# Ghostish/Open3DSOT

Measured on AMD Instinct MI355X. Metric: template/search pairs/sec (fwd+bwd), BAT KITTI-Car 512/1024 pts, higher is better.
Workload: dtype f32; 1 GPU; BAT_Car.yaml KITTI-Car, template 512 / search 1024 pts, batch 48 per GPU, fwd+bwd+Adam, fp32; global_batch=48, parallelism=dp1, fused_kernels=True, hip_graph=True, rccl_world_size=1

## Files before the change

### open3dsot_amd/csrc/mlp.hip

```cpp
#include "mlp_common.hpp"

#include <mutex>
#include <unordered_set>

bool o3d_direct_ok(int M, int K, int P);
int o3d_direct_fwd(const float* X, const float* W, const float* in_scale, const float* in_shift, int B, int Cin,
                   int Cout, int P, float* Y, float* part, const float* stat_c, const float* w, const int32_t* meta,
                   long start1, int tile, hipStream_t st);
int o3d_direct_dgrad(const float* dN, const float* pk, int ns,
                     const float* Y, const float* A1, const float* A2, const float* A3, const float* Wt, int B,
                     int Cin, int Cout, int P, const float* Yprev, const float* scale_p, const float* shift_p,
                     const float* mean_p, float* dNprev, float* part, const float* w, const int32_t* meta,
                     long start1, int tile, hipStream_t st);

namespace {


constexpr int BN_POS = 128;
constexpr int BK = 16;
constexpr int LDMK = BK + 4;
constexpr int WBK = 32;
constexpr int WLD = WBK + 4;

template <int CH, bool A_MK, bool B_MK>
// ... 623 lines not shown
        const int p = (ch - (int)b * chunks_per_b) * WBK + 4 * c4;
#pragma unroll
        for (int i = 0; i < 4; ++i) {
            const int co = co0 + r0 + 32 * i;
            if (co < a.Cout) ra[i] = load_dy_raw<POOLED>(a.dy, b, co, a.Cout, a.P, p);
            const int ci = ci0 + r0 + 32 * i;
            float4 v = make_float4(0.f, 0.f, 0.f, 0.f);
            float c0 = 0.f, c1 = 0.f;
            if (ci < a.Cin) {
                v = *reinterpret_cast<const float4*>(&a.X[(b * a.Cin + ci) * a.P + p]);
                if (XFORM) { c0 = a.in_scale[ci]; c1 = a.in_shift[ci]; }
            }
            rb[i] = v; rc0[i] = c0; rc1[i] = c1;
        }
    };
    auto store_chunk = [&](int buf) {
#pragma unroll
        for (int i = 0; i < 4; ++i) {
            const int co = co0 + r0 + 32 * i;
            *reinterpret_cast<float4*>(&As(buf)[(r0 + 32 * i) * WLD + 4 * c4]) =
                co < a.Cout ? finish_dy<POOLED>(ra[i]) : make_float4(0.f, 0.f, 0.f, 0.f);
            const int ci = ci0 + r0 + 32 * i;
            float4 v = rb[i];
            if (XFORM) {
                if (ci < a.Cin) {
                    const float sc = rc0[i], sh = rc1[i];
                    v.x = fmaxf(fmaf(v.x, sc, sh), 0.f); v.y = fmaxf(fmaf(v.y, sc, sh), 0.f);
                    v.z = fmaxf(fmaf(v.z, sc, sh), 0.f); v.w = fmaxf(fmaf(v.w, sc, sh), 0.f);
                }
            }
            *reinterpret_cast<float4*>(&Bs(buf)[(r0 + 32 * i) * WLD + 4 * c4]) = v;
        }
    };

    f32x16 acc[2][2];
#pragma unroll
    for (int i = 0; i < 2; ++i)
#pragma unroll
        for (int j = 0; j < 2; ++j)
#pragma unroll
            for (int r = 0; r < 16; ++r) acc[i][j][r] = 0.f;

    if (c_begin < c_end) {
        load_chunk(c_begin);
        store_chunk(0);
        __syncthreads();
        for (int ch = c_begin; ch < c_end; ++ch) {
            const int t = ch - c_begin;
            if (ch + 1 < c_end) load_chunk(ch + 1);
            mma_chunk<WBK, true, true>(As(t & 1), WLD, Bs(t & 1), WLD, wm0, wn0, l31, h, acc);
            if (ch + 1 < c_end) store_chunk((t + 1) & 1);
            __syncthreads();
        }
    }
    float* dst = a.part + (long)slice * a.Cout * a.Cin;
#pragma unroll
    for (int tm = 0; tm < 2; ++tm)
#pragma unroll
        for (int r = 0; r < 16; ++r) {
            const int co = co0 + wm0 + 32 * tm + acc_row(r, h);
            if (co >= a.Cout) continue;
#pragma unroll
            for (int tn = 0; tn < 2; ++tn) {
                const int ci = ci0 + wn0 + 32 * tn + l31;
                if (ci < a.Cin) dst[(long)co * a.Cin + ci] = acc[tm][tn][r];
            }
        }
}

__global__ __launch_bounds__(256) void wgrad_reduce_kernel(const float* __restrict__ part, int nslices,
                                                           int per, long n, float* __restrict__ out) {
    const long i = (long)blockIdx.x * 256 + threadIdx.x;
    if (i >= n) return;
    const int z0 = blockIdx.y * per;
    int z1 = z0 + per;
    if (z1 > nslices) z1 = nslices;
    float s = 0.f;
#pragma unroll 8
    for (int z = z0; z < z1; ++z) s += part[(long)z * n + i];
    out[(long)blockIdx.y * n + i] = s;
}

__global__ __launch_bounds__(256) void wgrad_reduce1_kernel(const float* __restrict__ part, int nslices, long n,
                                                            float* __restrict__ out) {
    __shared__ float sh[8][32];
    const int col = threadIdx.x & 31, grp = threadIdx.x >> 5;
    const long i = (long)blockIdx.x * 32 + col;
    const int per = (nslices + 7) / 8, z0 = grp * per;
    int z1 = z0 + per;
    if (z1 > nslices) z1 = nslices;
    float s0 = 0.f, s1 = 0.f, s2 = 0.f, s3 = 0.f;
    if (i < n) {
        int z = z0;
        for (; z + 3 < z1; z += 4) {
            s0 += part[(long)z * n + i]; s1 += part[(long)(z + 1) * n + i];
            s2 += part[(long)(z + 2) * n + i]; s3 += part[(long)(z + 3) * n + i];
        }
        for (; z < z1; ++z) s0 += part[(long)z * n + i];
    }
    sh[grp][col] = (s0 + s1) + (s2 + s3);
    __syncthreads();
    if (grp == 0 && i < n) {
        float t = 0.f;
#pragma unroll
        for (int g = 0; g < 8; ++g) t += sh[g][col];
        out[i] = t;
    }
}

template <typename K, typename... A>
int launch(K kernel, dim3 grid, dim3 block, size_t lds, hipStream_t s, A... args) {
    if (lds > 48 * 1024) {
        static std::mutex mu;
        static std::unordered_set<const void*> done;
        std::lock_guard<std::mutex> lock(mu);
        const void* key = reinterpret_cast<const void*>(kernel);
        if (!done.count(key)) {
            if (hipFuncSetAttribute(key, hipFuncAttributeMaxDynamicSharedMemorySize, (int)lds) != hipSuccess)
                return O3D_ELAUNCH;
            done.insert(key);
        }
    }
    hipLaunchKernelGGL(kernel, grid, block, lds, s, args...);
    return o3d_launch_status();
}

inline size_t fwd_lds(int BM) { return sizeof(float) * (2 * BM * LDMK + 2 * BK * BN_POS); }
inline size_t dgrad_lds(int BM) {
    size_t stage = sizeof(float) * (2 * BK * BM + 2 * BK * BN_POS), red = sizeof(float) * 4 * BM;
    return stage > red ? stage : red;
}

template <bool XFORM>
int launch_fwd(const FwdArgs& a, hipStream_t s) {
    const int tiles = a.B * (a.P / BN_POS);
    if (a.Cout > 128) {
        return launch(conv_fwd_kernel<256, XFORM>, dim3(tiles, o3d_cdiv(a.Cout, 256)), dim3(512),
                      fwd_lds(256), s, a);
    } else if (a.Cout > 64) {
        return launch(conv_fwd_kernel<128, XFORM>, dim3(tiles, 1), dim3(256), fwd_lds(128), s, a);
    }
    return launch(conv_fwd_kernel<64, XFORM>, dim3(tiles, 1), dim3(128), fwd_lds(64), s, a);
}

template <bool POOLED, int EPI>
int launch_dgrad(const DgradArgs& a, hipStream_t s) {
    const int tiles = a.B * (a.P / BN_POS);
    if (a.M > 128) {
        return launch(conv_dgrad_kernel<256, POOLED, EPI>, dim3(tiles, o3d_cdiv(a.M, 256)), dim3(512),
                      dgrad_lds(256), s, a);
    } else if (a.M > 64) {
        return launch(conv_dgrad_kernel<128, POOLED, EPI>, dim3(tiles, 1), dim3(256), dgrad_lds(128), s, a);
    }
    return launch(conv_dgrad_kernel<64, POOLED, EPI>, dim3(tiles, 1), dim3(128), dgrad_lds(64), s, a);
}

}

extern "C" int o3d_mlp_conv_fwd(const float* X, const float* W, const float* in_scale,
                                const float* in_shift, int B, int Cin, int Cout, int P, float* Y,
                                float* part, const float* stat_c, void* stream) {
    if (B <= 0 || Cin <= 0 || Cout <= 0 || P <= 0 || P % BN_POS != 0 || !X || !W || !Y) return O3D_EINVAL;
    if (o3d_direct_ok(Cout, Cin, P) && (in_scale == nullptr) == (in_shift == nullptr))
        return o3d_direct_fwd(X, W, in_scale, in_shift, B, Cin, Cout, P, Y, part, stat_c, nullptr, nullptr, 0,
                              part ? 128 : o3d_direct_tile((long)B * P, Cout, 0), o3d_stream(stream));
    FwdArgs a = {};
    a.X = X; a.W = W; a.Y = Y; a.in_scale = in_scale; a.in_shift = in_shift; a.part = part; a.stat_c = stat_c;
    a.B = B; a.Cin = Cin; a.Cout = Cout; a.P = P;
// ... 60 lines not shown
}

extern "C" int o3d_pool_bwd_partials_split(const float* dOut, const float* out, const float* yarg, const float* mean,
                                           int C, int npoint, int nsplit, float* part, const int32_t* arg, float* pk,
                                           void* stream) {
    if (C <= 0 || npoint <= 0 || nsplit <= 0 || nsplit > 64 || !dOut || !out || !yarg || !mean || !part || (pk && !arg))
        return O3D_EINVAL;
    hipLaunchKernelGGL(pool_bwd_partials_split_kernel, dim3(C, nsplit), dim3(256), 0, o3d_stream(stream), dOut, out, yarg,
                       mean, C, npoint, part, arg, reinterpret_cast<float2*>(pk));
    return o3d_launch_status();
}

static int fill_dy(DyArgs& d, const float* dN, const float* dOut, const float* out, const int32_t* arg,
                   const float* Y, const float* A1, const float* A2, const float* A3, int ns) {
    if (!Y || !A1 || !A2 || !A3) return O3D_EINVAL;
    if (!dN && (!dOut || !out || !arg || ns <= 0 || ns % 4 != 0)) return O3D_EINVAL;
    d.dN = dN; d.dOut = dOut; d.out = out; d.arg = arg; d.Y = Y; d.A1 = A1; d.A2 = A2; d.A3 = A3;
    d.ns = ns > 0 ? ns : 4;
    return O3D_OK;
}

extern "C" int o3d_mlp_conv_dgrad(const float* dN, const float* dOut, const float* out, const int32_t* arg,
                                  int ns, const float* Y, const float* A1, const float* A2, const float* A3,
                                  const float* W, int B, int Cin, int Cout, int P,
                                  const float* Yprev, const float* scale_p, const float* shift_p,
                                  const float* mean_p, float* dNprev, float* part, void* stream) {
    if (B <= 0 || Cin <= 0 || Cout <= 0 || P <= 0 || P % BN_POS != 0 || !W || !Yprev || !scale_p ||
        !shift_p || !mean_p || !dNprev || !part)
        return O3D_EINVAL;
    DgradArgs a = {};
    if (fill_dy(a.dy, dN, dOut, out, arg, Y, A1, A2, A3, ns) != O3D_OK) return O3D_EINVAL;
    a.W = W; a.B = B; a.Cin = Cin; a.Cout = Cout; a.P = P; a.c_lo = 0; a.M = Cin;
    a.Yprev = Yprev; a.scale_p = scale_p; a.shift_p = shift_p; a.mean_p = mean_p; a.dNprev = dNprev; a.part = part;
    return dN ? launch_dgrad<false, 0>(a, o3d_stream(stream)) : launch_dgrad<true, 0>(a, o3d_stream(stream));
}

extern "C" int o3d_mlp_conv_dgrad_wt(const float* dN, const float* dOut, const float* out, const int32_t* arg,
                                     int ns, const float* Y, const float* A1, const float* A2, const float* A3,
                                     const float* W, const float* Wt, const float* pk, int B, int Cin, int Cout,
                                     int P, const float* Yprev, const float* scale_p, const float* shift_p,
                                     const float* mean_p, float* dNprev, float* part, void* stream) {
    if (Wt && o3d_direct_ok(Cin, Cout, P) && B > 0 && Yprev && scale_p && shift_p && mean_p && dNprev && part &&
        Y && A1 && A2 && A3 && (dN || (pk && ns > 0 && ns % 4 == 0)))
        return o3d_direct_dgrad(dN, pk, ns, Y, A1, A2, A3, Wt, B, Cin, Cout, P, Yprev, scale_p, shift_p,
                                mean_p, dNprev, part, nullptr, nullptr, 0, 128, o3d_stream(stream));
    return o3d_mlp_conv_dgrad(dN, dOut, out, arg, ns, Y, A1, A2, A3, W, B, Cin, Cout, P, Yprev, scale_p, shift_p,
                              mean_p, dNprev, part, stream);
}

extern "C" int o3d_mlp_conv_fwd_c(const float* X, const float* W, const float* in_scale, const float* in_shift,
                                  int Cin, int Cout, long ldp, const float* w, const int32_t* meta, long start1,
                                  int tile, float* Y, float* part, const float* stat_c, void* stream) {
    if (!X || !W || !Y || !w || !meta || !in_scale || !in_shift || ldp <= 0 || ldp > 0x7fffffff ||
        !o3d_direct_ok(Cout, Cin, (int)ldp) || (tile != 64 && tile != 128))
        return O3D_EINVAL;
    return o3d_direct_fwd(X, W, in_scale, in_shift, 1, Cin, Cout, (int)ldp, Y, part, stat_c, w, meta, start1, tile,
                          o3d_stream(stream));
}

extern "C" int o3d_mlp_conv_dgrad_c(const float* dN, const float* Y, const float* A1, const float* A2,
                                    const float* A3, const float* Wt, int Cin, int Cout, long ldp, const float* w,
                                    const int32_t* meta, long start1, int tile, const float* Yprev,
                                    const float* scale_p,
                                    const float* shift_p, const float* mean_p, float* dNprev, float* part,
                                    void* stream) {
    if (!dN || !Y || !A1 || !A2 || !A3 || !Wt || !w || !meta || !Yprev || !scale_p || !shift_p || !mean_p ||
        !dNprev || !part || ldp <= 0 || ldp > 0x7fffffff || !o3d_direct_ok(Cin, Cout, (int)ldp) ||
        (tile != 64 && tile != 128))
        return O3D_EINVAL;
    return o3d_direct_dgrad(dN, nullptr, 4, Y, A1, A2, A3, Wt, 1, Cin, Cout, (int)ldp, Yprev, scale_p, shift_p,
                            mean_p, dNprev, part, w, meta, start1, tile, o3d_stream(stream));
}

extern "C" int o3d_mlp_conv_dgrad_plain(const float* dN, const float* Y, const float* A1, const float* A2,
                                        const float* A3, const float* W, int B, int Cin, int Cout, int P,
                                        float* dX, void* stream) {
    if (B <= 0 || Cin <= 0 || Cout <= 0 || P <= 0 || P % BN_POS != 0 || !W || !dN || !dX) return O3D_EINVAL;
    DgradArgs a = {};
    if (fill_dy(a.dy, dN, nullptr, nullptr, nullptr, Y, A1, A2, A3, 4) != O3D_OK) return O3D_EINVAL;
    a.W = W; a.B = B; a.Cin = Cin; a.Cout = Cout; a.P = P; a.c_lo = 0; a.M = Cin; a.dNprev = dX;
    return launch_dgrad<false, 2>(a, o3d_stream(stream));
}

void o3d_wgrad_reduce(const float* part, int nslices, long n, float* dW, hipStream_t s) {
    hipLaunchKernelGGL(wgrad_reduce1_kernel, dim3(o3d_cdiv(n, 32)), dim3(256), 0, s, part, nslices, n, dW);
}

extern "C" int o3d_mlp_conv_wgrad(const float* dN, const float* dOut, const float* out, const int32_t* arg,
                                  int ns, const float* Y, const float* A1, const float* A2, const float* A3,
                                  const float* X, const float* in_scale, const float* in_shift,
                                  int B, int Cin, int Cout, int P, int nslices, float* part, float* dW,
                                  void* stream) {
    if (B <= 0 || Cin <= 0 || Cout <= 0 || P <= 0 || P % WBK != 0 || nslices <= 0 || !X || !part || !dW)
        return O3D_EINVAL;
    WgradArgs a = {};
    if (fill_dy(a.dy, dN, dOut, out, arg, Y, A1, A2, A3, ns) != O3D_OK) return O3D_EINVAL;
    a.X = X; a.in_scale = in_scale; a.in_shift = in_shift;
    a.B = B; a.Cin = Cin; a.Cout = Cout; a.P = P;
    a.total_chunks = B * (P / WBK);
    a.chunks_per_block = (a.total_chunks + nslices - 1) / nslices;
    a.part = part;
    a.tiles_ci = o3d_cdiv(Cin, 128); a.tiles_co = o3d_cdiv(Cout, 128); a.nslices = nslices;
    const dim3 grid(a.tiles_ci * a.tiles_co * nslices), block(256);
    const size_t lds = sizeof(float) * 4 * 128 * WLD;
    hipStream_t s = o3d_stream(stream);
    int rc;
    const bool pooled = dN == nullptr;
    if (in_scale) {
        rc = pooled ? launch(conv_wgrad_kernel<true, true>, grid, block, lds, s, a)
                    : launch(conv_wgrad_kernel<false, true>, grid, block, lds, s, a);
    } else {
        rc = pooled ? launch(conv_wgrad_kernel<true, false>, grid, block, lds, s, a)
                    : launch(conv_wgrad_kernel<false, false>, grid, block, lds, s, a);
    }
    if (rc != O3D_OK) return rc;
    o3d_wgrad_reduce(part, nslices, (long)Cout * Cin, dW, s);
    return o3d_launch_status();
}
```

### open3dsot_amd/csrc/mlp_common.hpp

```cpp
#pragma once
#include "o3d_common.hpp"

typedef float f32x16 __attribute__((ext_vector_type(16)));

__device__ __forceinline__ f32x16 mfma32(float a, float b, f32x16 c) {
    return __builtin_amdgcn_mfma_f32_32x32x2f32(a, b, c, 0, 0, 0);
}

__device__ __forceinline__ int acc_row(int r, int h) { return (r & 3) + 8 * (r >> 2) + 4 * h; }

__device__ __forceinline__ void reduce_scatter32(float (&x)[32], int l31) {
#pragma unroll
    for (int m = 16; m >= 1; m >>= 1) {
        const bool up = (l31 & m) != 0;
#pragma unroll
        for (int v = 0; v < m; ++v) {
            float lo = x[v], hi = x[v + m];
            asm volatile("" : "+v"(lo), "+v"(hi));
            const float keep = up ? hi : lo;
            const float send = up ? lo : hi;
            x[v] = keep + __shfl_xor(send, m, 64);
        }
    }
}

struct TailPlan { int full, R, f; };
__host__ __device__ __forceinline__ TailPlan tail_plan(int T, int S, int cap) {
    TailPlan p = {T, 0, 1};
    if (S <= 0 || T <= 0) return p;
    const int R = T % S;
    if (R == 0) return p;
    const int f = 4 * R <= S ? 4 : (2 * R <= S ? 2 : 1);
    if (f == 1 || T + R * (f - 1) > cap) return p;
    p.full = T - R; p.R = R; p.f = f;
    return p;
}
extern "C" int o3d_direct_tail_slots(int M);
```

### open3dsot_amd/csrc/mlp_wgrad.hip

```cpp
#include "mlp_common.hpp"

namespace {

struct Wgrad2Args {
    const float* dN;
    const float2* pk;
    int ns;
    const float* Y;
    const float* A1; const float* A2; const float* A3;
    const float* X;
    const float* in_scale; const float* in_shift;
    int B, Cin, Cout, P;
    int chunks_per_block, total_chunks, nslices;
    float* part;
    const float* w;
    const int32_t* meta;
    long start1;
};

template <int TM, int TN, int POOLED>
__device__ __forceinline__ void wgrad2_body(const Wgrad2Args& a, const int bid, float* smem) {
    constexpr int WM = TM / 64, WN = TN / 64, WK = 4 / (WM * WN);
    constexpr int CP = (TM + TN == 128) ? 64 : 32;
    constexpr int LD = CP + 4;
    constexpr int F = CP / 4;
    constexpr int RPP = 256 / F;
    constexpr int PA = TM / RPP, PB = TN / RPP;
    constexpr int NG = CP / WK / 8;
    auto As = [&](int buf) -> float* { return smem + buf * ((TM + TN) * LD); };
    auto Bs = [&](int buf) -> float* { return smem + buf * ((TM + TN) * LD) + TM * LD; };

    const int tid = threadIdx.x, lane = tid & 63, wave = tid >> 6;
    const int l31 = lane & 31, h = lane >> 5;
    const int wk = wave / (WM * WN), wmn = wave - wk * (WM * WN);
    const int wm0 = (wmn / WN) * 64, wn0 = (wmn % WN) * 64;
    const int tiles_ci = a.Cin / TN, ntile = tiles_ci * (a.Cout / TM);
    int tile_id, slice;
    if ((a.nslices & 7) == 0) {
        const int xcd = bid & 7, local = bid >> 3;
        tile_id = local % ntile;
        slice = (local / ntile) * 8 + xcd;
    } else {
        tile_id = bid % ntile;
        slice = bid / ntile;
    }
    const int ci0 = (tile_id % tiles_ci) * TN, co0 = (tile_id / tiles_ci) * TM;
    int c_begin, c_end;
    int seg = 0;
    long col0 = 0;
    if (a.meta) {
        const int n0 = a.meta[0] / CP, n1 = a.start1 > 0 ? a.meta[4] / CP : 0;
        int nsl0 = a.nslices;
        if (n1 > 0) {
            nsl0 = (int)(((long)a.nslices * n0 + (n0 + n1) / 2) / (n0 + n1));
            nsl0 = nsl0 < 1 ? 1 : (nsl0 > a.nslices - 1 ? a.nslices - 1 : nsl0);
        }
        seg = slice >= nsl0 ? 1 : 0;
        const int nsl = seg ? a.nslices - nsl0 : nsl0, ls = seg ? slice - nsl0 : slice, n = seg ? n1 : n0;
        const int per = (n + nsl - 1) / nsl;
        c_begin = ls * per;
        c_end = c_begin + per < n ? c_begin + per : n;
        col0 = seg ? a.start1 : 0;
    } else {
        c_begin = slice * a.chunks_per_block;
        c_end = c_begin + a.chunks_per_block < a.total_chunks ? c_begin + a.chunks_per_block : a.total_chunks;
    }
    const float* A1 = a.A1 + (seg ? a.Cout : 0);
    const float* A2 = a.A2 + (seg ? a.Cout : 0);
    const float* A3 = a.A3 + (seg ? a.Cout : 0);
    const bool plain_x = a.in_scale == nullptr;
    const float* in_scale = plain_x ? nullptr : a.in_scale + (seg ? a.Cin : 0);
    const float* in_shift = plain_x ? nullptr : a.in_shift + (seg ? a.Cin : 0);
    const float x_floor = plain_x ? -INFINITY : 0.f;
    const int chunks_per_b = a.P / CP;
    const int r0 = tid / F, c4 = tid % F;
    const int np = POOLED == 1 ? a.P / a.ns : 1;

    float ka1[PA], ka2[PA], ka3[PA], ksc[PB], ksh[PB];
#pragma unroll
    for (int i = 0; i < PA; ++i) {
        const int co = co0 + r0 + RPP * i;
        ka1[i] = A1[co]; ka2[i] = A2[co]; ka3[i] = A3[co];
    }
#pragma unroll
    for (int i = 0; i < PB; ++i) {
        const int ci = ci0 + r0 + RPP * i;
        ksc[i] = plain_x ? 1.f : in_scale[ci]; ksh[i] = plain_x ? 0.f : in_shift[ci];
    }

    float4 rg[PA], ry[PA], rx[PB];
    float4 rw = make_float4(1.f, 1.f, 1.f, 1.f);
    int rk = 0;
    auto load_chunk = [&](int chl) {
        const long chg = col0 / CP + chl;
        const long b = chg / chunks_per_b;
        const int p = (int)(chg - b * chunks_per_b) * CP + 4 * c4;
        if (a.w) rw = *reinterpret_cast<const float4*>(&a.w[b * a.P + p]);
#pragma unroll
        for (int i = 0; i < PA; ++i) {
            const long row = b * a.Cout + co0 + r0 + RPP * i;
            ry[i] = *reinterpret_cast<const float4*>(&a.Y[row * a.P + p]);
            if (POOLED) {
                const int j = p / a.ns;
                const float2 t = a.pk[row * np + j];
                rg[i].x = t.x; rg[i].y = t.y;
                rk = p - j * a.ns;
            } else {
                rg[i] = *reinterpret_cast<const float4*>(&a.dN[row * a.P + p]);
            }
        }
#pragma unroll
        for (int i = 0; i < PB; ++i)
            rx[i] = *reinterpret_cast<const float4*>(&a.X[(b * a.Cin + ci0 + r0 + RPP * i) * a.P + p]);
    };
    auto store_chunk = [&](int buf) {
#pragma unroll
        for (int i = 0; i < PA; ++i) {
            float4 g;
            if (POOLED) {
                const int ak = __float_as_int(rg[i].y);
                const float go = rg[i].x;
                g.x = (rk + 0 == ak) ? go : 0.f; g.y = (rk + 1 == ak) ? go : 0.f;
                g.z = (rk + 2 == ak) ? go : 0.f; g.w = (rk + 3 == ak) ? go : 0.f;
            } else {
                g = rg[i];
            }
            float4 o;
            o.x = fmaf(ka1[i], g.x, rw.x * fmaf(ka2[i], ry[i].x, ka3[i])); o.y = fmaf(ka1[i], g.y, rw.y * fmaf(ka2[i], ry[i].y, ka3[i]));
            o.z = fmaf(ka1[i], g.z, rw.z * fmaf(ka2[i], ry[i].z, ka3[i])); o.w = fmaf(ka1[i], g.w, rw.w * fmaf(ka2[i], ry[i].w, ka3[i]));
            *reinterpret_cast<float4*>(&As(buf)[(r0 + RPP * i) * LD + 4 * c4]) = o;
        }
#pragma unroll
        for (int i = 0; i < PB; ++i) {
            float4 v = rx[i];
            v.x = fmaxf(fmaf(v.x, ksc[i], ksh[i]), x_floor); v.y = fmaxf(fmaf(v.y, ksc[i], ksh[i]), x_floor);
            v.z = fmaxf(fmaf(v.z, ksc[i], ksh[i]), x_floor); v.w = fmaxf(fmaf(v.w, ksc[i], ksh[i]), x_floor);
            *reinterpret_cast<float4*>(&Bs(buf)[(r0 + RPP * i) * LD + 4 * c4]) = v;
        }
    };

    f32x16 acc[2][2];
#pragma unroll
    for (int i = 0; i < 2; ++i)
#pragma unroll
        for (int j = 0; j < 2; ++j)
#pragma unroll
            for (int r = 0; r < 16; ++r) acc[i][j][r] = 0.f;

    if (c_begin < c_end) {
        load_chunk(c_begin);
        store_chunk(0);
        __syncthreads();
        for (int ch = c_begin; ch < c_end; ++ch) {
            const int t = ch - c_begin;
            if (ch + 1 < c_end) load_chunk(ch + 1);
            const float* A_ = As(t & 1) + wk * (CP / WK);
            const float* B_ = Bs(t & 1) + wk * (CP / WK);
#pragma unroll
            for (int g = 0; g < NG; ++g) {
                float av[2][4], bv[2][4];
#pragma unroll
                for (int u = 0; u < 2; ++u) {
                    const float4 x = *reinterpret_cast<const float4*>(&A_[(wm0 + 32 * u + l31) * LD + 8 * g + 4 * h]);
                    av[u][0] = x.x; av[u][1] = x.y; av[u][2] = x.z; av[u][3] = x.w;
                    const float4 y = *reinterpret_cast<const float4*>(&B_[(wn0 + 32 * u + l31) * LD + 8 * g + 4 * h]);
                    bv[u][0] = y.x; bv[u][1] = y.y; bv[u][2] = y.z; bv[u][3] = y.w;
                }
#pragma unroll
                for (int s = 0; s < 4; ++s)
#pragma unroll
                    for (int tm = 0; tm < 2; ++tm)
#pragma unroll
                        for (int tn = 0; tn < 2; ++tn) acc[tm][tn] = mfma32(av[tm][s], bv[tn][s], acc[tm][tn]);
            }
            if (ch + 1 < c_end) store_chunk((t + 1) & 1);
            __syncthreads();
        }
    }
    float* dst = a.part + (long)(slice * WK + wk) * a.Cout * a.Cin;
#pragma unroll
    for (int tm = 0; tm < 2; ++tm)
#pragma unroll
        for (int r = 0; r < 16; ++r) {
            const int co = co0 + wm0 + 32 * tm + acc_row(r, h);
#pragma unroll
            for (int tn = 0; tn < 2; ++tn) dst[(long)co * a.Cin + ci0 + wn0 + 32 * tn + l31] = acc[tm][tn][r];
        }
}

template <int TM, int TN, int POOLED>
__global__ __launch_bounds__(256) void wgrad2_kernel(Wgrad2Args a) {
    extern __shared__ __attribute__((aligned(16))) float smem[];
    wgrad2_body<TM, TN, POOLED>(a, blockIdx.x, smem);
}

constexpr int WG_MAXJOBS = 8;
struct Wgrad2Group {
    Wgrad2Args job[WG_MAXJOBS];
    int first[WG_MAXJOBS + 1];
    int kind[WG_MAXJOBS];
    int njobs;
};

__device__ __forceinline__ void row_sum_body(const Wgrad2Args& a, const int bid, float* smem) {
    const float* g = a.dN + (long)bid * a.P;
    float s = 0.f;
    for (long p = 4L * threadIdx.x; p < a.P; p += 1024) {
        const float4 v = *reinterpret_cast<const float4*>(g + p);
        s += (v.x + v.y) + (v.z + v.w);
    }
#pragma unroll
    for (int off = 32; off >= 1; off >>= 1) s += __shfl_xor(s, off, 64);
    if ((threadIdx.x & 63) == 0) smem[threadIdx.x >> 6] = s;
    __syncthreads();
    if (threadIdx.x == 0) a.part[bid] = (smem[0] + smem[1]) + (smem[2] + smem[3]);
}

__global__ __launch_bounds__(256) void wgrad2_group_kernel(Wgrad2Group g) {
    extern __shared__ __attribute__((aligned(16))) float smem[];
    int j = 0;
    while (j + 1 < g.njobs && (int)blockIdx.x >= g.first[j + 1]) ++j;
    const int bid = blockIdx.x - g.first[j];
    switch (g.kind[j]) {
        case 0: wgrad2_body<128, 128, 0>(g.job[j], bid, smem); break;
        case 1: wgrad2_body<128, 64, 0>(g.job[j], bid, smem); break;
        case 2: wgrad2_body<64, 128, 0>(g.job[j], bid, smem); break;
        case 3: wgrad2_body<64, 64, 0>(g.job[j], bid, smem); break;
        default: row_sum_body(g.job[j], bid, smem); break;
    }
}

struct ReduceGroup {
    const float* part[WG_MAXJOBS]; float* out[WG_MAXJOBS];
    long n[WG_MAXJOBS]; int nslices[WG_MAXJOBS]; int first[WG_MAXJOBS + 1]; int njobs;
    int ld[WG_MAXJOBS], orows[WG_MAXJOBS], ocols[WG_MAXJOBS];
};

__global__ __launch_bounds__(256) void wgrad_reduce_group_kernel(ReduceGroup r) {
    __shared__ float sh[8][32];
    int j = 0;
    while (j + 1 < r.njobs && (int)blockIdx.x >= r.first[j + 1]) ++j;
    const float* __restrict__ part = r.part[j];
    const long n = r.n[j];
    const int nslices = r.nslices[j];
    const int col = threadIdx.x & 31, grp = threadIdx.x >> 5;
    const long i = (long)(blockIdx.x - r.first[j]) * 32 + col;
    const int per = (nslices + 7) / 8, z0 = grp * per;
    int z1 = z0 + per;
    if (z1 > nslices) z1 = nslices;
    float s0 = 0.f, s1 = 0.f, s2 = 0.f, s3 = 0.f;
    if (i < n) {
        int z = z0;
        for (; z + 3 < z1; z += 4) {
            s0 += part[(long)z * n + i]; s1 += part[(long)(z + 1) * n + i];
            s2 += part[(long)(z + 2) * n + i]; s3 += part[(long)(z + 3) * n + i];
        }
        for (; z < z1; ++z) s0 += part[(long)z * n + i];
    }
    sh[grp][col] = (s0 + s1) + (s2 + s3);
    __syncthreads();
    if (grp == 0 && i < n) {
        float t = 0.f;
// ... 165 lines not shown
                        for (int tm = 0; tm < 2; ++tm)
#pragma unroll
                            for (int tn = 0; tn < 2; ++tn) acc[tm][tn] = mfma32(av[tm][s], bv[tn][s], acc[tm][tn]);
                }
            }
            if (dactive) {
                f32x16 d;
#pragma unroll
                for (int r = 0; r < 16; ++r) d[r] = 0.f;
                const float* Bd = A_ + 32 * dpt + l31;
#pragma unroll
                for (int g = 0; g < GD; ++g) {
                    const float b0 = Bd[(8 * g + 4 * h + 0) * LD], b1 = Bd[(8 * g + 4 * h + 1) * LD];
                    const float b2 = Bd[(8 * g + 4 * h + 2) * LD], b3 = Bd[(8 * g + 4 * h + 3) * LD];
                    d = mfma32(wt[g].x, b0, d);
                    d = mfma32(wt[g].y, b1, d);
                    d = mfma32(wt[g].z, b2, d);
                    d = mfma32(wt[g].w, b3, d);
                }
                const long q = (col0 / CP + ch) * CP + 32 * dpt + l31;
#pragma unroll
                for (int r = 0; r < 16; ++r) {
                    const int row = acc_row(r, h);
                    const float xt = B_[(dci + row) * LD + 32 * dpt + l31];
                    const float gq = xt > 0.f ? d[r] : 0.f;
                    a.dX[(long)(dci + row) * a.P + q] = gq;
                    sacc[r] += gq;
                    sacc[16 + r] = fmaf(gq, xt, sacc[16 + r]);
                }
            }
            if (ch + 1 < c_end) store_chunk((t + 1) & 1);
            __syncthreads();
        }
    }
    float* dst = a.part_w + (long)(slice * WK + wk) * TM * TN;
#pragma unroll
    for (int tm = 0; tm < 2; ++tm)
#pragma unroll
        for (int r = 0; r < 16; ++r) {
            const int co = wm0 + 32 * tm + acc_row(r, h);
#pragma unroll
            for (int tn = 0; tn < 2; ++tn) dst[(long)co * TN + 32 * tn + l31] = acc[tm][tn][r];
        }
    if (dactive) {
        reduce_scatter32(sacc, l31);
        const int ci = dci + acc_row(l31 & 15, h);
        const int which = l31 >> 4;
        const float other = __shfl_xor(sacc[0], 16, 64);
        const float s1 = which ? other : sacc[0], s2x = which ? sacc[0] : other;
        const float sc = in_scale[ci], beta = fmaf(sc, in_mean[ci], in_shift[ci]);
        float s2 = sc != 0.f ? (s2x - beta * s1) / sc : 0.f;
        if (sc == 0.f && which) {
            asm volatile("s_waitcnt vmcnt(0)" ::: "memory");
            const float mu = in_mean[ci];
            float t2 = 0.f;
            for (int ch = c_begin; ch < c_end; ++ch) {
                const long qb = (col0 / CP + ch) * CP + 32 * dpt;
                for (int j = 0; j < 32; ++j)
                    t2 = fmaf(a.dX[(long)ci * a.P + qb + j], a.X[(long)ci * a.P + qb + j] - mu, t2);
            }
            s2 = t2;
        }
        const long rows = (long)a.nslices * NPT, row = (long)slice * NPT + dpt;
        float* mine = a.part_s + ((long)seg * rows + row) * 2 * TN;
        float* theirs = a.part_s + ((long)(1 - seg) * rows + row) * 2 * TN;
        mine[which * TN + ci] = which ? s2 : s1;
        theirs[which * TN + ci] = 0.f;
    }
}

template <int TM>
int launch_fused_bwd(const FusedBwdArgs& a, hipStream_t s) {
    constexpr int CP = (TM + 64 == 128) ? 64 : 32;
    const size_t lds = sizeof(float) * 2 * (TM + 64) * (CP + 4);
    const void* fn = reinterpret_cast<const void*>(fused_bwd_kernel<TM>);
    if (lds > 48 * 1024 && hipFuncSetAttribute(fn, hipFuncAttributeMaxDynamicSharedMemorySize, (int)lds) != hipSuccess)
        return -3;
    hipLaunchKernelGGL((fused_bwd_kernel<TM>), dim3(a.nslices), dim3(256), lds, s, a);
    return hipGetLastError() == hipSuccess ? 0 : -3;
}

}

void o3d_wgrad_reduce(const float* part, int nslices, long n, float* dW, hipStream_t s);

static void wgrad2_plan(int Cin, int Cout, int B, int P, int& TM, int& TN, int& WK, int& CP, int& nsl) {
    TM = Cout % 128 == 0 ? 128 : 64;
    TN = Cin % 128 == 0 ? 128 : 64;
    WK = 4 / ((TM / 64) * (TN / 64));
    CP = (TM + TN == 128) ? 64 : 32;
    const int ntile = (Cout / TM) * (Cin / TN);
    const long total = (long)B * (P / CP);
    constexpr int wgs = 512;
    nsl = wgs / ntile;
    if (nsl < 8) nsl = 8;
    while (nsl > 8 && total / nsl < 4) nsl -= 8;
    if (nsl > total) nsl = (int)total;
}

extern "C" long o3d_mlp_conv_wgrad2_scratch(int B, int Cin, int Cout, int P) {
    if (Cin <= 0 || Cout <= 0 || Cin % 64 || Cout % 64 || P <= 0 || P % 64 || B <= 0) return -1;
    int TM, TN, WK, CP, nsl;
    wgrad2_plan(Cin, Cout, B, P, TM, TN, WK, CP, nsl);
    return ((long)nsl * WK + 16) * Cout * Cin;
}

static int wgrad2_impl(const float* dN, const float* pk, int ns, const float* Y, const float* A1, const float* A2,
                       const float* A3, const float* X, const float* in_scale, const float* in_shift, int B, int Cin,
                       int Cout, int P, const float* w, const int32_t* meta, long start1, float* scratch, float* dW,
                       void* stream) {
    if (B <= 0 || Cin <= 0 || Cout <= 0 || Cin % 64 || Cout % 64 || P <= 0 || P % 64 || !Y || !A1 || !A2 || !A3 ||
        !X || (in_scale == nullptr) != (in_shift == nullptr) || !scratch || !dW || (!dN && (!pk || ns < 4 || ns % 4)))
        return O3D_EINVAL;
    int TM, TN, WK, CP, nsl;
    wgrad2_plan(Cin, Cout, B, P, TM, TN, WK, CP, nsl);
    Wgrad2Args a = {};
    a.dN = dN; a.pk = reinterpret_cast<const float2*>(pk); a.ns = ns > 0 ? ns : 4; a.Y = Y;
    a.A1 = A1; a.A2 = A2; a.A3 = A3; a.X = X; a.in_scale = in_scale; a.in_shift = in_shift;
    a.B = B; a.Cin = Cin; a.Cout = Cout; a.P = P;
    a.total_chunks = B * (P / CP);
    a.chunks_per_block = (a.total_chunks + nsl - 1) / nsl;
    a.nslices = nsl;
    a.part = scratch;
    a.w = w; a.meta = meta; a.start1 = start1;
    hipStream_t s = o3d_stream(stream);
    int rc;
    if (TM == 128 && TN == 128) rc = launch_wgrad2<128, 128>(a, s);
    else if (TM == 128)         rc = launch_wgrad2<128, 64>(a, s);
    else if (TN == 128)         rc = launch_wgrad2<64, 128>(a, s);
    else                        rc = launch_wgrad2<64, 64>(a, s);
    if (rc != O3D_OK) return rc;
    const long n = (long)Cout * Cin;
    o3d_wgrad_reduce(scratch, nsl * WK, n, dW, s);
    return o3d_launch_status();
}

extern "C" int o3d_mlp_conv_wgrad2(const float* dN, const float* pk, int ns, const float* Y, const float* A1,
                                   const float* A2, const float* A3, const float* X, const float* in_scale,
                                   const float* in_shift, int B, int Cin, int Cout, int P, float* scratch,
                                   float* dW, void* stream) {
    return wgrad2_impl(dN, pk, ns, Y, A1, A2, A3, X, in_scale, in_shift, B, Cin, Cout, P, nullptr, nullptr, 0, scratch,
                       dW, stream);
}

extern "C" int o3d_mlp_conv_wgrad2_c(const float* dN, const float* Y, const float* A1, const float* A2,
                                     const float* A3, const float* X, const float* in_scale, const float* in_shift,
                                     int Cin, int Cout, long ldp, const float* w, const int32_t* meta, long start1,
                                     float* scratch, float* dW, void* stream) {
    if (!dN || !w || !meta || ldp <= 0 || ldp > 0x7fffffff || start1 < 0 || start1 % 256 != 0) return O3D_EINVAL;
    return wgrad2_impl(dN, nullptr, 4, Y, A1, A2, A3, X, in_scale, in_shift, 1, Cin, Cout, (int)ldp, w, meta, start1,
                       scratch, dW, stream);
}


extern "C" int o3d_mlp_conv_wgrad2_group(const o3d_wgrad_job* jobs, int njobs, void* stream) {
    if (!jobs || njobs < 1 || njobs > WG_MAXJOBS) return O3D_EINVAL;
    Wgrad2Group g = {};
    ReduceGroup r = {};
    g.njobs = r.njobs = njobs;
    size_t lds = 0;
    int nblk = 0, rblk = 0;
    for (int i = 0; i < njobs; ++i) {
        const o3d_wgrad_job& q = jobs[i];
        if (q.dN && !q.X && !q.Y && q.dW && q.Cout > 0 && q.P > 0 && q.P % 4 == 0 && q.P <= 0x7fffffff) {
            Wgrad2Args& a = g.job[i];
            a.dN = q.dN; a.P = (int)q.P; a.Cout = q.Cout; a.part = q.dW;
            g.kind[i] = 4;
            g.first[i] = nblk;
            nblk += q.Cout;
            r.part[i] = q.dW; r.out[i] = q.dW; r.n[i] = 0; r.nslices[i] = 0; r.ld[i] = 1; r.orows[i] = r.ocols[i] = 0;
            r.first[i] = rblk;
            continue;
        }
        if (!q.dN || !q.Y || !q.A1 || !q.A2 || !q.A3 || !q.X || (q.in_scale == nullptr) != (q.in_shift == nullptr) ||
            !q.scratch || !q.dW || q.Cin <= 0 || q.Cout <= 0 || q.Cin % 64 || q.Cout % 64 || q.P <= 0 || q.P % 64 ||
            q.P > 0x7fffffff)
            return O3D_EINVAL;
        int TM, TN, WK, CP, nsl;
        wgrad2_plan(q.Cin, q.Cout, 1, (int)q.P, TM, TN, WK, CP, nsl);
        Wgrad2Args& a = g.job[i];
        a.dN = q.dN; a.ns = 4; a.Y = q.Y; a.A1 = q.A1; a.A2 = q.A2; a.A3 = q.A3; a.X = q.X;
        a.in_scale = q.in_scale; a.in_shift = q.in_shift; a.B = 1; a.Cin = q.Cin; a.Cout = q.Cout; a.P = (int)q.P;
        a.total_chunks = (int)(q.P / CP);
        a.chunks_per_block = (a.total_chunks + nsl - 1) / nsl;
        a.nslices = nsl;
        a.part = q.scratch;
        g.kind[i] = TM == 128 ? (TN == 128 ? 0 : 1) : (TN == 128 ? 2 : 3);
        g.first[i] = nblk;
        nblk += (q.Cout / TM) * (q.Cin / TN) * nsl;
        const size_t l = sizeof(float) * 2 * (TM + TN) * (CP + 4);
        lds = l > lds ? l : lds;
        if (q.out_rows < 0 || q.out_rows > q.Cout || q.out_cols < 0 || q.out_cols > q.Cin) return O3D_EINVAL;
        r.part[i] = q.scratch; r.out[i] = q.dW; r.n[i] = (long)q.Cout * q.Cin; r.nslices[i] = nsl * WK;
        r.ld[i] = q.Cin; r.orows[i] = q.out_rows > 0 ? q.out_rows : q.Cout; r.ocols[i] = q.out_cols > 0 ? q.out_cols : q.Cin;
        r.first[i] = rblk;
        rblk += o3d_cdiv(r.n[i], 32);
    }
    g.first[njobs] = nblk;
    r.first[njobs] = rblk;
    static const bool attr_ok = hipFuncSetAttribute(reinterpret_cast<const void*>(wgrad2_group_kernel),
                                                    hipFuncAttributeMaxDynamicSharedMemorySize, 80 * 1024) == hipSuccess;
    if (!attr_ok || lds > 80 * 1024) return O3D_ELAUNCH;
    hipStream_t s = o3d_stream(stream);
    if (lds < 16) lds = 16;
    hipLaunchKernelGGL(wgrad2_group_kernel, dim3(nblk), dim3(256), lds, s, g);
    if (rblk > 0) hipLaunchKernelGGL(wgrad_reduce_group_kernel, dim3(rblk), dim3(256), 0, s, r);
    return o3d_launch_status();
}


static int fused_bwd_slices(int Cout, long P) {
    constexpr int wgs = 256;
    const int CP = (Cout + 64 == 128) ? 64 : 32;
    const long total = P / CP;
    int nsl = wgs;
    while (nsl > 8 && total / nsl < 4) nsl -= 8;
    if (nsl > total) nsl = (int)total;
    return nsl < 1 ? 1 : nsl;
}
static bool fused_bwd_ok(int Cin, int Cout, long P) {
    return Cin == 64 && (Cout == 64 || Cout == 128) && P > 0 && P % 64 == 0 && P <= 0x7fffffff;
}

extern "C" int o3d_mlp_conv_bwd_fused_rows(int Cin, int Cout, long P) {
    return fused_bwd_ok(Cin, Cout, P) ? fused_bwd_slices(Cout, P) * (Cout == 64 ? 2 : 1) : -1;
}
extern "C" long o3d_mlp_conv_bwd_fused_scratch(int Cin, int Cout, long P) {
    return fused_bwd_ok(Cin, Cout, P) ? (long)fused_bwd_slices(Cout, P) * (4 / (Cout / 64)) * Cout * Cin : -1;
}

extern "C" int o3d_mlp_conv_bwd_fused_c(const float* dN, const float* Y, const float* A1, const float* A2, const float* A3,
                                        const float* X, const float* in_scale, const float* in_shift, const float* in_mean,
                                        const float* Wt, int Cin, int Cout, long ldp, const float* w, const int32_t* meta,
                                        long start1, float* scratch, float* dW, float* part_s, float* dNprev, void* stream) {
    if (!dN || !Y || !A1 || !A2 || !A3 || !X || !in_scale || !in_shift || !in_mean || !Wt || !scratch || !dW || !part_s ||
        !dNprev || !fused_bwd_ok(Cin, Cout, ldp) || (meta != nullptr) != (w != nullptr) || start1 < 0 || start1 % 256 != 0)
        return O3D_EINVAL;
    const int CP = (Cout + 64 == 128) ? 64 : 32;
    const int nsl = fused_bwd_slices(Cout, ldp);
    FusedBwdArgs a = {};
    a.dN = dN; a.Y = Y; a.A1 = A1; a.A2 = A2; a.A3 = A3; a.X = X; a.in_scale = in_scale; a.in_shift = in_shift;
    a.in_mean = in_mean; a.Wt = Wt; a.Cin = Cin; a.Cout = Cout; a.P = (int)ldp;
    a.total_chunks = (int)(ldp / CP);
    a.chunks_per_block = (a.total_chunks + nsl - 1) / nsl;
    a.nslices = nsl;
    a.w = w; a.meta = meta; a.start1 = start1; a.part_w = scratch; a.part_s = part_s; a.dX = dNprev;
    hipStream_t s = o3d_stream(stream);
    const int rc = Cout == 64 ? launch_fused_bwd<64>(a, s) : launch_fused_bwd<128>(a, s);
    if (rc != 0) return O3D_ELAUNCH;
    const long n = (long)Cout * Cin;
    o3d_wgrad_reduce(scratch, nsl * (4 / (Cout / 64)), n, dW, s);
    return o3d_launch_status();
}
```

Before: 9208 pairs/s.

## Interleave wgrad staging with MFMA, fold k-groups in LDS, skip dead slices

Restructures the wgrad2 kernel so global loads and LDS stores for the next chunk are split into passes interleaved between MFMA steps, with double-buffered fragment reads, to hide memory latency. The per-warp k-split partial sums are now folded in shared memory before writing one slab per slice, shrinking scratch traffic and the reduce kernel's input. Slices are also planned with a minimum chunk count so padded/empty slices exit early and the reducer only sums live slabs. This adds register pressure, extra syncs and scheduling barriers, and more complex indexing.

```diff
diff --git a/open3dsot_amd/csrc/mlp.hip b/open3dsot_amd/csrc/mlp.hip
--- a/open3dsot_amd/csrc/mlp.hip
+++ b/open3dsot_amd/csrc/mlp.hip
@@ -729,8 +729,15 @@
 }
 
 __global__ __launch_bounds__(256) void wgrad_reduce1_kernel(const float* __restrict__ part, int nslices, long n,
-                                                            float* __restrict__ out) {
+                                                            float* __restrict__ out, const int32_t* __restrict__ meta,
+                                                            long start1, int cp) {
     __shared__ float sh[8][32];
+    if (meta) {
+        int n0, n1;
+        wgrad_live_chunks(meta, start1, cp, n0, n1);
+        const WgradSlicePlan pl = wgrad_slice_plan(nslices, n0, n1);
+        nslices = pl.used0 + pl.used1;
+    }
     const int col = threadIdx.x & 31, grp = threadIdx.x >> 5;
     const long i = (long)blockIdx.x * 32 + col;
     const int per = (nslices + 7) / 8, z0 = grp * per;
@@ -957,8 +964,9 @@
     return launch_dgrad<false, 2>(a, o3d_stream(stream));
 }
 
-void o3d_wgrad_reduce(const float* part, int nslices, long n, float* dW, hipStream_t s) {
-    hipLaunchKernelGGL(wgrad_reduce1_kernel, dim3(o3d_cdiv(n, 32)), dim3(256), 0, s, part, nslices, n, dW);
+void o3d_wgrad_reduce(const float* part, int nslices, long n, float* dW, hipStream_t s, const int32_t* meta, long start1,
+                      int cp) {
+    hipLaunchKernelGGL(wgrad_reduce1_kernel, dim3(o3d_cdiv(n, 32)), dim3(256), 0, s, part, nslices, n, dW, meta, start1, cp);
 }
 
 extern "C" int o3d_mlp_conv_wgrad(const float* dN, const float* dOut, const float* out, const int32_t* arg,
@@ -989,6 +997,6 @@
                     : launch(conv_wgrad_kernel<false, false>, grid, block, lds, s, a);
     }
     if (rc != O3D_OK) return rc;
-    o3d_wgrad_reduce(part, nslices, (long)Cout * Cin, dW, s);
+    o3d_wgrad_reduce(part, nslices, (long)Cout * Cin, dW, s, nullptr, 0, 0);
     return o3d_launch_status();
 }
diff --git a/open3dsot_amd/csrc/mlp_common.hpp b/open3dsot_amd/csrc/mlp_common.hpp
--- a/open3dsot_amd/csrc/mlp_common.hpp
+++ b/open3dsot_amd/csrc/mlp_common.hpp
@@ -35,4 +35,40 @@
     p.full = T - R; p.R = R; p.f = f;
     return p;
 }
+
+constexpr int WGRAD_MIN_CHUNKS = 4;
+struct WgradSlicePlan { int nsl0, used0, used1; };
+__host__ __device__ __forceinline__ WgradSlicePlan wgrad_slice_plan(int nslices, int n0, int n1) {
+    int nsl0 = nslices;
+    if (n1 > 0) {
+        nsl0 = (int)(((long)nslices * n0 + (n0 + n1) / 2) / (n0 + n1));
+        nsl0 = nsl0 < 1 ? 1 : (nsl0 > nslices - 1 ? nslices - 1 : nsl0);
+    }
+    const int nsl1 = nslices - nsl0;
+    const int w0 = n0 / WGRAD_MIN_CHUNKS < 1 ? 1 : n0 / WGRAD_MIN_CHUNKS;
+    const int w1 = n1 / WGRAD_MIN_CHUNKS < 1 ? 1 : n1 / WGRAD_MIN_CHUNKS;
+    WgradSlicePlan p;
+    p.nsl0 = nsl0;
+    p.used0 = n0 == 0 ? 0 : (w0 < nsl0 ? w0 : nsl0);
+    p.used1 = n1 == 0 ? 0 : (w1 < nsl1 ? w1 : nsl1);
+    return p;
+}
+struct WgradSlice { int seg, c_begin, c_end, slab; };
+__host__ __device__ __forceinline__ WgradSlice wgrad_slice(const WgradSlicePlan& p, int n0, int n1, int slice) {
+    WgradSlice s;
+    s.seg = slice >= p.nsl0 ? 1 : 0;
+    const int ls = s.seg ? slice - p.nsl0 : slice, used = s.seg ? p.used1 : p.used0, n = s.seg ? n1 : n0;
+    s.c_begin = s.c_end = 0;
+    s.slab = -1;
+    if (ls >= used) return s;
+    s.c_begin = (int)((long)ls * n / used);
+    s.c_end = (int)((long)(ls + 1) * n / used);
+    s.slab = s.seg ? p.used0 + ls : ls;
+    return s;
+}
+__host__ __device__ __forceinline__ void wgrad_live_chunks(const int32_t* meta, long start1, int cp, int& n0, int& n1) {
+    n0 = meta[0] > 0 ? meta[0] / cp : 0;
+    n1 = start1 > 0 && meta[4] > 0 ? meta[4] / cp : 0;
+}
+
 extern "C" int o3d_direct_tail_slots(int M);
diff --git a/open3dsot_amd/csrc/mlp_wgrad.hip b/open3dsot_amd/csrc/mlp_wgrad.hip
--- a/open3dsot_amd/csrc/mlp_wgrad.hip
+++ b/open3dsot_amd/csrc/mlp_wgrad.hip
@@ -46,20 +46,14 @@
     }
     const int ci0 = (tile_id % tiles_ci) * TN, co0 = (tile_id / tiles_ci) * TM;
     int c_begin, c_end;
-    int seg = 0;
+    int seg = 0, slab = slice;
     long col0 = 0;
     if (a.meta) {
-        const int n0 = a.meta[0] / CP, n1 = a.start1 > 0 ? a.meta[4] / CP : 0;
-        int nsl0 = a.nslices;
-        if (n1 > 0) {
-            nsl0 = (int)(((long)a.nslices * n0 + (n0 + n1) / 2) / (n0 + n1));
-            nsl0 = nsl0 < 1 ? 1 : (nsl0 > a.nslices - 1 ? a.nslices - 1 : nsl0);
-        }
-        seg = slice >= nsl0 ? 1 : 0;
-        const int nsl = seg ? a.nslices - nsl0 : nsl0, ls = seg ? slice - nsl0 : slice, n = seg ? n1 : n0;
-        const int per = (n + nsl - 1) / nsl;
-        c_begin = ls * per;
-        c_end = c_begin + per < n ? c_begin + per : n;
+        int n0, n1;
+        wgrad_live_chunks(a.meta, a.start1, CP, n0, n1);
+        const WgradSlice sl = wgrad_slice(wgrad_slice_plan(a.nslices, n0, n1), n0, n1, slice);
+        if (sl.slab < 0) return;
+        seg = sl.seg; slab = sl.slab; c_begin = sl.c_begin; c_end = sl.c_end;
         col0 = seg ? a.start1 : 0;
     } else {
         c_begin = slice * a.chunks_per_block;
@@ -88,37 +82,57 @@
         ksc[i] = plain_x ? 1.f : in_scale[ci]; ksh[i] = plain_x ? 0.f : in_shift[ci];
     }
 
+    constexpr int K = PA + PB, KPG = K / NG;
+    static_assert(K % NG == 0 && KPG <= 4, "staging passes must divide over the k groups, at most one per MFMA step");
     float4 rg[PA], ry[PA], rx[PB];
-    float4 rw = make_float4(1.f, 1.f, 1.f, 1.f);
-    int rk = 0;
-    auto load_chunk = [&](int chl) {
-        const long chg = col0 / CP + chl;
-        const long b = chg / chunks_per_b;
-        const int p = (int)(chg - b * chunks_per_b) * CP + 4 * c4;
-        if (a.w) rw = *reinterpret_cast<const float4*>(&a.w[b * a.P + p]);
-#pragma unroll
-        for (int i = 0; i < PA; ++i) {
-            const long row = b * a.Cout + co0 + r0 + RPP * i;
-            ry[i] = *reinterpret_cast<const float4*>(&a.Y[row * a.P + p]);
+    float4 rw = make_float4(1.f, 1.f, 1.f, 1.f), rw_next = rw;
+    long lb = 0;
+    int lp = 0, lch = c_begin;
+    {
+        const long chg = col0 / CP + c_begin;
+        lb = chg / chunks_per_b;
+        lp = (int)(chg - lb * chunks_per_b) * CP;
+    }
+    auto next_chunk = [&]() {
+        if (lch + 1 < c_end) {
+            ++lch;
+            lp += CP;
+            if (lp == a.P) { lp = 0; ++lb; }
+        }
+    };
+    const long tA = (long)(co0 + r0) * a.P + 4 * c4, tB = (long)(ci0 + r0) * a.P + 4 * c4;
+    const float* const pY = a.Y + tA;
+    const float* const pG = POOLED ? nullptr : a.dN + tA;
+    const float* const pX = a.X + tB;
+    auto load_w = [&]() {
+        if (a.w) rw_next = *reinterpret_cast<const float4*>(&a.w[lb * a.P + lp + 4 * c4]);
+    };
+    auto load_pass = [&](int k) {
+        if (k < PA) {
+            const int i = k;
+            const long off = (lb * a.Cout + RPP * i) * a.P + lp;
+            ry[i] = *reinterpret_cast<const float4*>(pY + off);
             if (POOLED) {
+                const int p = lp + 4 * c4;
+                const long row = lb * a.Cout + co0 + r0 + RPP * i;
                 const int j = p / a.ns;
                 const float2 t = a.pk[row * np + j];
                 rg[i].x = t.x; rg[i].y = t.y;
-                rk = p - j * a.ns;
+                rg[i].z = __int_as_float(p - j * a.ns);
             } else {
-                rg[i] = *reinterpret_cast<const float4*>(&a.dN[row * a.P + p]);
+                rg[i] = *reinterpret_cast<const float4*>(pG + off);
             }
-        }
-#pragma unroll
-        for (int i = 0; i < PB; ++i)
-            rx[i] = *reinterpret_cast<const float4*>(&a.X[(b * a.Cin + ci0 + r0 + RPP * i) * a.P + p]);
+        } else {
+            const int i = k - PA;
+            rx[i] = *reinterpret_cast<const float4*>(pX + (lb * a.Cin + RPP * i) * a.P + lp);
+        }
     };
-    auto store_chunk = [&](int buf) {
-#pragma unroll
-        for (int i = 0; i < PA; ++i) {
+    auto store_pass = [&](int k, int buf) {
+        if (k < PA) {
+            const int i = k;
             float4 g;
             if (POOLED) {
-                const int ak = __float_as_int(rg[i].y);
+                const int ak = __float_as_int(rg[i].y), rk = __float_as_int(rg[i].z);
                 const float go = rg[i].x;
                 g.x = (rk + 0 == ak) ? go : 0.f; g.y = (rk + 1 == ak) ? go : 0.f;
                 g.z = (rk + 2 == ak) ? go : 0.f; g.w = (rk + 3 == ak) ? go : 0.f;
@@ -129,9 +143,8 @@
             o.x = fmaf(ka1[i], g.x, rw.x * fmaf(ka2[i], ry[i].x, ka3[i])); o.y = fmaf(ka1[i], g.y, rw.y * fmaf(ka2[i], ry[i].y, ka3[i]));
             o.z = fmaf(ka1[i], g.z, rw.z * fmaf(ka2[i], ry[i].z, ka3[i])); o.w = fmaf(ka1[i], g.w, rw.w * fmaf(ka2[i], ry[i].w, ka3[i]));
             *reinterpret_cast<float4*>(&As(buf)[(r0 + RPP * i) * LD + 4 * c4]) = o;
-        }
-#pragma unroll
-        for (int i = 0; i < PB; ++i) {
+        } else {
+            const int i = k - PA;
             float4 v = rx[i];
             v.x = fmaxf(fmaf(v.x, ksc[i], ksh[i]), x_floor); v.y = fmaxf(fmaf(v.y, ksc[i], ksh[i]), x_floor);
             v.z = fmaxf(fmaf(v.z, ksc[i], ksh[i]), x_floor); v.w = fmaxf(fmaf(v.w, ksc[i], ksh[i]), x_floor);
@@ -148,36 +161,86 @@
             for (int r = 0; r < 16; ++r) acc[i][j][r] = 0.f;
 
     if (c_begin < c_end) {
-        load_chunk(c_begin);
-        store_chunk(0);
+        load_w();
+#pragma unroll
+        for (int k = 0; k < K; ++k) load_pass(k);
+        rw = rw_next;
+        next_chunk();
+        load_w();
+#pragma unroll
+        for (int k = 0; k < K; ++k) { store_pass(k, 0); load_pass(k); }
         __syncthreads();
         for (int ch = c_begin; ch < c_end; ++ch) {
             const int t = ch - c_begin;
-            if (ch + 1 < c_end) load_chunk(ch + 1);
             const float* A_ = As(t & 1) + wk * (CP / WK);
             const float* B_ = Bs(t & 1) + wk * (CP / WK);
-#pragma unroll
-            for (int g = 0; g < NG; ++g) {
-                float av[2][4], bv[2][4];
+            rw = rw_next;
+            next_chunk();
+            load_w();
+            float av[2][2][4], bv[2][2][4];
+            auto read_frag = [&](int g) {
 #pragma unroll
                 for (int u = 0; u < 2; ++u) {
                     const float4 x = *reinterpret_cast<const float4*>(&A_[(wm0 + 32 * u + l31) * LD + 8 * g + 4 * h]);
-                    av[u][0] = x.x; av[u][1] = x.y; av[u][2] = x.z; av[u][3] = x.w;
+                    av[g & 1][u][0] = x.x; av[g & 1][u][1] = x.y; av[g & 1][u][2] = x.z; av[g & 1][u][3] = x.w;
                     const float4 y = *reinterpret_cast<const float4*>(&B_[(wn0 + 32 * u + l31) * LD + 8 * g + 4 * h]);
-                    bv[u][0] = y.x; bv[u][1] = y.y; bv[u][2] = y.z; bv[u][3] = y.w;
+                    bv[g & 1][u][0] = y.x; bv[g & 1][u][1] = y.y; bv[g & 1][u][2] = y.z; bv[g & 1][u][3] = y.w;
                 }
-#pragma unroll
-                for (int s = 0; s < 4; ++s)
+            };
+            read_frag(0);
+#pragma unroll
+            for (int g = 0; g < NG; ++g) {
+                if (g + 1 < NG) read_frag(g + 1);
+#pragma unroll
+                for (int s = 0; s < 4; ++s) {
 #pragma unroll
                     for (int tm = 0; tm < 2; ++tm)
 #pragma unroll
-                        for (int tn = 0; tn < 2; ++tn) acc[tm][tn] = mfma32(av[tm][s], bv[tn][s], acc[tm][tn]);
+                        for (int tn = 0; tn < 2; ++tn)
+                            acc[tm][tn] = mfma32(av[g & 1][tm][s], bv[g & 1][tn][s], acc[tm][tn]);
+#pragma unroll
+                    for (int j = 0; j < KPG; ++j)
+                        if (j * 4 / KPG == s) {
+                            store_pass(g * KPG + j, (t + 1) & 1);
+                            load_pass(g * KPG + j);
+                        }
+                    __builtin_amdgcn_sched_barrier(0);
+                }
             }
-            if (ch + 1 < c_end) store_chunk((t + 1) & 1);
             __syncthreads();
         }
     }
-    float* dst = a.part + (long)(slice * WK + wk) * a.Cout * a.Cin;
+    if (WK > 1) {
+        float4* fold = reinterpret_cast<float4*>(smem);
+        if (wk > 0) {
+            float4* f = fold + ((wk - 1) * (WM * WN) + wmn) * 16 * 64 + lane;
+#pragma unroll
+            for (int tm = 0; tm < 2; ++tm)
+#pragma unroll
+                for (int tn = 0; tn < 2; ++tn)
+#pragma unroll
+                    for (int q = 0; q < 4; ++q)
+                        f[((tm * 2 + tn) * 4 + q) * 64] = make_float4(acc[tm][tn][4 * q], acc[tm][tn][4 * q + 1],
+                                                                      acc[tm][tn][4 * q + 2], acc[tm][tn][4 * q + 3]);
+        }
+        __syncthreads();
+        if (wk > 0) return;
+#pragma unroll
+        for (int k = 1; k < WK; ++k) {
+            const float4* f = fold + ((k - 1) * (WM * WN) + wmn) * 16 * 64 + lane;
+#pragma unroll
+            for (int tm = 0; tm < 2; ++tm)
+#pragma unroll
+                for (int tn = 0; tn < 2; ++tn)
+#pragma unroll
+                    for (int q = 0; q < 4; ++q) {
+                        const float4 v = f[((tm * 2 + tn) * 4 + q) * 64];
+                        acc[tm][tn][4 * q] += v.x; acc[tm][tn][4 * q + 1] += v.y;
+                        acc[tm][tn][4 * q + 2] += v.z; acc[tm][tn][4 * q + 3] += v.w;
+                    }
+        }
+    }
+    float* dst = a.part + (long)slab * a.Cout * a.Cin;
 #pragma unroll
     for (int tm = 0; tm < 2; ++tm)
 #pragma unroll
@@ -509,7 +572,8 @@
 
 }
 
-void o3d_wgrad_reduce(const float* part, int nslices, long n, float* dW, hipStream_t s);
+void o3d_wgrad_reduce(const float* part, int nslices, long n, float* dW, hipStream_t s, const int32_t* meta, long start1,
+                      int cp);
 
 static void wgrad2_plan(int Cin, int Cout, int B, int P, int& TM, int& TN, int& WK, int& CP, int& nsl) {
     TM = Cout % 128 == 0 ? 128 : 64;
@@ -529,7 +593,7 @@
     if (Cin <= 0 || Cout <= 0 || Cin % 64 || Cout % 64 || P <= 0 || P % 64 || B <= 0) return -1;
     int TM, TN, WK, CP, nsl;
     wgrad2_plan(Cin, Cout, B, P, TM, TN, WK, CP, nsl);
-    return ((long)nsl * WK + 16) * Cout * Cin;
+    return (long)nsl * Cout * Cin;
 }
 
 static int wgrad2_impl(const float* dN, const float* pk, int ns, const float* Y, const float* A1, const float* A2,
@@ -558,7 +622,7 @@
     else                        rc = launch_wgrad2<64, 64>(a, s);
     if (rc != O3D_OK) return rc;
     const long n = (long)Cout * Cin;
-    o3d_wgrad_reduce(scratch, nsl * WK, n, dW, s);
+    o3d_wgrad_reduce(scratch, nsl, n, dW, s, meta, start1, CP);
     return o3d_launch_status();
 }
 
@@ -618,7 +682,7 @@
         const size_t l = sizeof(float) * 2 * (TM + TN) * (CP + 4);
         lds = l > lds ? l : lds;
         if (q.out_rows < 0 || q.out_rows > q.Cout || q.out_cols < 0 || q.out_cols > q.Cin) return O3D_EINVAL;
-        r.part[i] = q.scratch; r.out[i] = q.dW; r.n[i] = (long)q.Cout * q.Cin; r.nslices[i] = nsl * WK;
+        r.part[i] = q.scratch; r.out[i] = q.dW; r.n[i] = (long)q.Cout * q.Cin; r.nslices[i] = nsl;
         r.ld[i] = q.Cin; r.orows[i] = q.out_rows > 0 ? q.out_rows : q.Cout; r.ocols[i] = q.out_cols > 0 ? q.out_cols : q.Cin;
         r.first[i] = rblk;
         rblk += o3d_cdiv(r.n[i], 32);
@@ -676,6 +740,6 @@
     const int rc = Cout == 64 ? launch_fused_bwd<64>(a, s) : launch_fused_bwd<128>(a, s);
     if (rc != 0) return O3D_ELAUNCH;
     const long n = (long)Cout * Cin;
-    o3d_wgrad_reduce(scratch, nsl * (4 / (Cout / 64)), n, dW, s);
+    o3d_wgrad_reduce(scratch, nsl * (4 / (Cout / 64)), n, dW, s, nullptr, 0, 0);
     return o3d_launch_status();
 }
```

Result: no change. 9279 pairs/s, median of 6 (+0.8%).
